# vinits5/bullet-envs

Measured on AMD Instinct MI355X. Metric: env-steps/sec (whole node), 16-link snake, 4096 envs/GPU, higher is better.
Workload: dtype f32

## Files before the change

### bullet-envs_amd/csrc/snk_dynamics.hpp

```cpp
#pragma once
#include "snk_lds.hpp"
#include "snk_model.hpp"
#include "snk_wave.hpp"

namespace snk {

template <class LT>
__device__ void fk_vel(LT& L, const DevModel& M, int lane) {
    constexpr int N = LT::kN;
    const float* bs = L.base();
    float qx = bs[3], qy = bs[4], qz = bs[5], qw = bs[6];
    float dd = qx * qx + qy * qy + qz * qz + qw * qw;
    float s2 = 2.0f / dd;
    float xs = qx * s2, ys = qy * s2, zs = qz * s2;
    float wx = qw * xs, wy = qw * ys, wz = qw * zs;
    float xx = qx * xs, xy = qx * ys, xz = qx * zs, yy = qy * ys, yz = qy * zs, zz = qz * zs;
    float Rp[9] = {1 - (yy + zz), xy - wz, xz + wy, xy + wz, 1 - (xx + zz), yz - wx, xz - wy, yz + wx, 1 - (xx + yy)};
    f3 op = ld3(bs), wp = ld3(bs + 7), vp = ld3(bs + 10);
    if (lane == 0) {
#pragma unroll
        for (int i = 0; i < 9; i++) L.R[0][i] = Rp[i];
        st3(L.o[0], op); st3(L.w[0], wp); st3(L.v[0], vp);
        st3(L.r[0], mk3(0, 0, 0)); st3(L.ax[0], mk3(0, 0, 0));
#pragma unroll
        for (int i = 0; i < 6; i++) L.zeta[0][i] = 0.f;
    }
    float snv = 0.f, csv = 1.f;
    if (lane < N) sincosf(L.q()[lane], &snv, &csv);
#pragma unroll 4
    for (int b = 1; b <= N; b++) {
        const float* Rf = M.Rfix[b];
        float T[9];
#pragma unroll
        for (int i = 0; i < 3; i++)
#pragma unroll
            for (int j = 0; j < 3; j++)
                T[3 * i + j] = Rp[3 * i] * Rf[j] + Rp[3 * i + 1] * Rf[3 + j] + Rp[3 * i + 2] * Rf[6 + j];
        float qdb = L.qd()[b - 1];
        const float sn = __int_as_float(__builtin_amdgcn_readlane(__float_as_int(snv), b - 1));
        const float cs = __int_as_float(__builtin_amdgcn_readlane(__float_as_int(csv), b - 1));
        float Rn[9];
#pragma unroll
        for (int i = 0; i < 3; i++) {
            Rn[3 * i + 0] = cs * T[3 * i] - sn * T[3 * i + 2];
            Rn[3 * i + 1] = T[3 * i + 1];
            Rn[3 * i + 2] = sn * T[3 * i] + cs * T[3 * i + 2];
        }
        f3 rb = mulRv(Rp, ld3(M.pfix[b]));
        f3 o = op + rb;
        f3 ax = mk3(T[1], T[4], T[7]);
        f3 w = wp + ax * qdb;
        f3 v = vp + cross(wp, rb);
        f3 za = cross(wp, ax) * qdb;
        f3 zl = cross(wp, cross(wp, rb));
        if (lane == 0) {
#pragma unroll
            for (int i = 0; i < 9; i++) L.R[b][i] = Rn[i];
            st3(L.o[b], o); st3(L.r[b], rb); st3(L.ax[b], ax); st3(L.w[b], w); st3(L.v[b], v);
            st3(&L.zeta[b][0], za); st3(&L.zeta[b][3], zl);
        }
#pragma unroll
        for (int i = 0; i < 9; i++) Rp[i] = Rn[i];
        op = o; wp = w; vp = v;
    }
    lds_sync();
}

template <class LT>
__device__ float mean_height(LT& L, const DevModel& M, int lane) {
    constexpr int N = LT::kN;
    float z = 0.f;
    if (lane == 0) z = L.o[0][2] + L.R[0][6] * M.hbase[0] + L.R[0][7] * M.hbase[1] + L.R[0][8] * M.hbase[2];
    else if (lane <= N) z = L.o[lane][2];
    return wave_sum<64>(z) * (1.0f / (N + 1));
}

template <class LT, bool FIRST>
__device__ void body_bias(LT& L, const DevModel& M, int lane) {
    constexpr int N = LT::kN;
    if (lane <= N) {
        const int b = lane;
        const float* R = L.R[b];
        f3 w = ld3(L.w[b]), v = ld3(L.v[b]);
        float m = M.mass[b];
        f3 cw = mulRv(R, ld3(M.com[b]));
        float Ibar[6];
        rotSym(R, M.Ib[b], Ibar);
        f3 pN = cross(w, mulSv(Ibar, w));
        f3 pF = cross(w, cross(w, cw)) * m;
        float Irw[6];
        rotSym(R, M.Irot[b], Irw);
        float nw = sqrtf(dot(w, w));
        pN = pN + mulSv(Irw, w) * (M.ang_damp + M.ang_damp * nw);
        const int ns = M.nsub[b];
        for (int s = 0; s < ns; s++) {
            f3 cs = mulRv(R, ld3(M.sub_c[b][s]));
            f3 vs = v + cross(w, cs);
            float nv = sqrtf(dot(vs, vs));
            f3 F = vs * (M.sub_m[b][s] * (M.lin_damp + M.lin_damp * nv));
            pF = pF + F;
            pN = pN + cross(cs, F);
        }
        if (FIRST) {
            f3 G = mk3(0.f, 0.f, m * M.gz);
            pF = pF - G;
            pN = pN - cross(cw, G);
            st3(L.cw[b], cw);
            float* IA = L.IA[b];
#pragma unroll
            for (int i = 0; i < 6; i++) IA[i] = Ibar[i];
            float hx = m * cw.x, hy = m * cw.y, hz = m * cw.z;
            IA[6] = 0.f; IA[7] = -hz; IA[8] = hy;
            IA[9] = hz;  IA[10] = 0.f; IA[11] = -hx;
            IA[12] = -hy; IA[13] = hx; IA[14] = 0.f;
            IA[15] = m; IA[16] = 0.f; IA[17] = 0.f; IA[18] = m; IA[19] = 0.f; IA[20] = m;
        } else {
            pN = pN - ld3(L.ext(b));
            pF = pF - ld3(L.ext(b) + 3);
        }
        st3(&L.p[b][0], pN);
        st3(&L.p[b][3], pF);
    }
}

template <class LT, bool FACTOR>
__device__ void aba_main(LT& L, const DevModel& M, int lane) {
    constexpr int N = LT::kN;
    float cA[6], cB[9], cC[6];
#pragma unroll
    for (int i = 0; i < 6; i++) { cA[i] = 0.f; cC[i] = 0.f; }
#pragma unroll
    for (int i = 0; i < 9; i++) cB[i] = 0.f;
    f3 cN = mk3(0, 0, 0), cF = mk3(0, 0, 0);
    for (int b = N; b >= 1; b--) {
        float A[6], B[9], C[6];
        float* IA = L.IA[b];
#pragma unroll
        for (int i = 0; i < 6; i++) { A[i] = IA[i]; C[i] = IA[15 + i]; }
#pragma unroll
        for (int i = 0; i < 9; i++) B[i] = IA[6 + i];
        if (FACTOR) {
#pragma unroll
            for (int i = 0; i < 6; i++) { A[i] += cA[i]; C[i] += cC[i]; }
#pragma unroll
            for (int i = 0; i < 9; i++) B[i] += cB[i];
        }
        f3 pN = ld3(&L.p[b][0]) + cN, pF = ld3(&L.p[b][3]) + cF;
        f3 ax = ld3(L.ax[b]);
        f3 Ua, Ub;
        float Dinv;
        if (FACTOR) {
            Ua = mulSv(A, ax);
            Ub = mk3(B[0] * ax.x + B[3] * ax.y + B[6] * ax.z, B[1] * ax.x + B[4] * ax.y + B[7] * ax.z,
                     B[2] * ax.x + B[5] * ax.y + B[8] * ax.z);
            Dinv = 1.0f / dot(ax, Ua);
        } else {
            Ua = ld3(L.Ua[b]); Ub = ld3(L.Ub[b]); Dinv = L.Dinv[b];
        }
        f3 za = ld3(&L.zeta[b][0]), zl = ld3(&L.zeta[b][3]);
        float u = L.tauj[b - 1] - dot(ax, pN);
        f3 tN = mulSv(A, za) + mk3(B[0] * zl.x + B[1] * zl.y + B[2] * zl.z, B[3] * zl.x + B[4] * zl.y + B[5] * zl.z,
                                   B[6] * zl.x + B[7] * zl.y + B[8] * zl.z);
        f3 tF = mk3(B[0] * za.x + B[3] * za.y + B[6] * za.z, B[1] * za.x + B[4] * za.y + B[7] * za.z,
                    B[2] * za.x + B[5] * za.y + B[8] * za.z) + mulSv(C, zl);
        float uz = dot(Ua, za) + dot(Ub, zl);
        float s = (u - uz) * Dinv;
        f3 paN = pN + tN + Ua * s, paF = pF + tF + Ub * s;
        f3 r = ld3(L.r[b]);
        cN = paN + cross(r, paF);
        cF = paF;
        if (lane == 0) {
            L.u[b] = u;
            if (FACTOR) {
#pragma unroll
                for (int i = 0; i < 6; i++) { IA[i] = A[i]; IA[15 + i] = C[i]; }
#pragma unroll
                for (int i = 0; i < 9; i++) IA[6 + i] = B[i];
                st3(L.Ua[b], Ua); st3(L.Ub[b], Ub); L.Dinv[b] = Dinv;
            }
        }
        if (FACTOR) {
            float ua[3] = {Ua.x, Ua.y, Ua.z}, ub[3] = {Ub.x, Ub.y, Ub.z};
            float Ap[6], Bp[9], Cp[6];
            Ap[0] = A[0] - ua[0] * ua[0] * Dinv; Ap[1] = A[1] - ua[0] * ua[1] * Dinv; Ap[2] = A[2] - ua[0] * ua[2] * Dinv;
            Ap[3] = A[3] - ua[1] * ua[1] * Dinv; Ap[4] = A[4] - ua[1] * ua[2] * Dinv; Ap[5] = A[5] - ua[2] * ua[2] * Dinv;
            Cp[0] = C[0] - ub[0] * ub[0] * Dinv; Cp[1] = C[1] - ub[0] * ub[1] * Dinv; Cp[2] = C[2] - ub[0] * ub[2] * Dinv;
            Cp[3] = C[3] - ub[1] * ub[1] * Dinv; Cp[4] = C[4] - ub[1] * ub[2] * Dinv; Cp[5] = C[5] - ub[2] * ub[2] * Dinv;
#pragma unroll
            for (int i = 0; i < 3; i++)
#pragma unroll
                for (int j = 0; j < 3; j++) Bp[3 * i + j] = B[3 * i + j] - ua[i] * ub[j] * Dinv;
            f3 c0 = cross(r, mk3(Cp[0], Cp[1], Cp[2]));
            f3 c1 = cross(r, mk3(Cp[1], Cp[3], Cp[4]));
            f3 c2 = cross(r, mk3(Cp[2], Cp[4], Cp[5]));
            float Bn[9] = {Bp[0] + c0.x, Bp[1] + c1.x, Bp[2] + c2.x, Bp[3] + c0.y, Bp[4] + c1.y, Bp[5] + c2.y,
                           Bp[6] + c0.z, Bp[7] + c1.z, Bp[8] + c2.z};
            f3 e0 = cross(r, mk3(Bp[0], Bp[1], Bp[2])), e1 = cross(r, mk3(Bp[3], Bp[4], Bp[5])),
               e2 = cross(r, mk3(Bp[6], Bp[7], Bp[8]));
            f3 g0 = cross(r, mk3(Bn[0], Bn[1], Bn[2])), g1 = cross(r, mk3(Bn[3], Bn[4], Bn[5])),
               g2 = cross(r, mk3(Bn[6], Bn[7], Bn[8]));
            cA[0] = Ap[0] + e0.x + g0.x;
            cA[1] = Ap[1] + e0.y + g1.x;
            cA[2] = Ap[2] + e0.z + g2.x;
            cA[3] = Ap[3] + e1.y + g1.y;
            cA[4] = Ap[4] + e1.z + g2.y;
            cA[5] = Ap[5] + e2.z + g2.z;
#pragma unroll
            for (int i = 0; i < 9; i++) cB[i] = Bn[i];
#pragma unroll
            for (int i = 0; i < 6; i++) cC[i] = Cp[i];
        }
    }
    f3 pN = ld3(&L.p[0][0]) + cN, pF = ld3(&L.p[0][3]) + cF;
    float p0[6] = {pN.x, pN.y, pN.z, pF.x, pF.y, pF.z};
    if (FACTOR) {
        float* IA = L.IA[0];
        float A[6], B[9], C[6];
#pragma unroll
        for (int i = 0; i < 6; i++) { A[i] = IA[i] + cA[i]; C[i] = IA[15 + i] + cC[i]; }
#pragma unroll
        for (int i = 0; i < 9; i++) B[i] = IA[6 + i] + cB[i];
        float G[6][6];
        G[0][0] = A[0]; G[0][1] = A[1]; G[0][2] = A[2]; G[1][1] = A[3]; G[1][2] = A[4]; G[2][2] = A[5];
        G[1][0] = A[1]; G[2][0] = A[2]; G[2][1] = A[4];
        G[3][3] = C[0]; G[3][4] = C[1]; G[3][5] = C[2]; G[4][4] = C[3]; G[4][5] = C[4]; G[5][5] = C[5];
        G[4][3] = C[1]; G[5][3] = C[2]; G[5][4] = C[4];
#pragma unroll
        for (int i = 0; i < 3; i++)
#pragma unroll
            for (int j = 0; j < 3; j++) { G[i][3 + j] = B[3 * i + j]; G[3 + j][i] = B[3 * i + j]; }
        float V[6][6];
#pragma unroll
        for (int i = 0; i < 6; i++)
#pragma unroll
            for (int j = 0; j < 6; j++) V[i][j] = (i == j) ? 1.f : 0.f;
#pragma unroll
        for (int k = 0; k < 6; k++) {
            float piv = 1.0f / G[k][k];
#pragma unroll
            for (int j = 0; j < 6; j++) { G[k][j] *= piv; V[k][j] *= piv; }
#pragma unroll
            for (int i = 0; i < 6; i++) {
                if (i != k) {
                    float f = G[i][k];
#pragma unroll
                    for (int j = 0; j < 6; j++) { G[i][j] -= f * G[k][j]; V[i][j] -= f * V[k][j]; }
                }
            }
        }
        if (lane == 0) {
#pragma unroll
            for (int i = 0; i < 6; i++)
#pragma unroll
                for (int j = 0; j < 6; j++) L.Inv0[6 * i + j] = V[i][j];
        }
        float a0[6];
#pragma unroll
        for (int i = 0; i < 6; i++) {
            float s = 0.f;
#pragma unroll
            for (int j = 0; j < 6; j++) s -= V[i][j] * p0[j];
            a0[i] = s;
        }
        if (lane == 0) {
#pragma unroll
            for (int i = 0; i < 6; i++) L.acc0[i] = a0[i];
        }
    } else {
        float a0[6];
#pragma unroll
        for (int i = 0; i < 6; i++) {
            float s = 0.f;
#pragma unroll
            for (int j = 0; j < 6; j++) s -= L.Inv0[6 * i + j] * p0[j];
            a0[i] = s;
        }
        if (lane == 0) {
#pragma unroll
            for (int i = 0; i < 6; i++) L.acc0[i] = a0[i];
        }
    }
    lds_sync();
    if (!FACTOR) return;
    f3 al = ld3(&L.acc0[0]), a = ld3(&L.acc0[3]);
    for (int b = 1; b <= N; b++) {
        f3 r = ld3(L.r[b]);
        f3 ap = a + cross(al, r) + ld3(&L.zeta[b][3]);
        f3 alp = al + ld3(&L.zeta[b][0]);
        float qdd = (L.u[b] - (dot(ld3(L.Ua[b]), alp) + dot(ld3(L.Ub[b]), ap))) * L.Dinv[b];
        al = alp + ld3(L.ax[b]) * qdd;
        a = ap;
        if (lane == 0) L.qdd[b - 1] = qdd;
    }
    lds_sync();
}

template <class LT>
__device__ __forceinline__ bool sensor_pass_needed(LT& L, const DevModel& M, int lane, float dv, const SensorHint& hint) {
    constexpr int N = LT::kN;
    constexpr int ND = N + 6;
    if (hint.always) return true;
    const float dt = M.dt;
    float e = 0.f, wgt = 0.f;
    if (lane < ND) {
        const float vold = lane < 6 ? L.base()[7 + lane] : L.qd()[lane - 6];
        const float x = fminf(fmaxf(vold + dv, -M.max_vel), M.max_vel);
        if (lane >= 6) e = L.targets[lane - 6] - (L.q()[lane - 6] + dt * x);
        wgt = fabsf(x) * ((lane >= 3 && lane < 6) ? 1.0f : 0.0639f * (N + 2));
    }
    const float se = wave_sum<64>(e * e);
    const float reach = dt * wave_sum<64>(wgt);
    const float tol = M.servo_tol * 1.001f;
    const bool sensor = !(se > tol * tol) || hint.counter_next > M.max_counter || !(hint.h_prev + reach < M.height_thr);
    return __builtin_amdgcn_readfirstlane(sensor ? 1 : 0) != 0;
}

}
```

### bullet-envs_amd/csrc/snk_pgs_v2.hpp

```cpp
#pragma once
#include "snk_contacts.hpp"
#include "snk_dynamics.hpp"
#include "snk_lds.hpp"
#include "snk_model.hpp"
#include "snk_selfcol.hpp"
#include "snk_wave.hpp"

namespace snk {


constexpr int kSlotNormal = 0;
constexpr int kSlotFric = 32;
constexpr int kSlots = 96;
constexpr int kAppMotor = 0;
constexpr int kAppNormal = 16;
constexpr int kAppFric = 80;
constexpr unsigned long long kLowMask = 0x00000000FFFFFFFFull;


struct ObsHit {
    bool hit;
    f3 P, n, dA, dB;
    float dist;
};
// ... 522 lines not shown
        "v_readlane_b32 %[s0], %[RJ], 31\n\t"
        SNK_REDUCE_12
        "v_readlane_b32 %[s2], %[RJ], 63\n\t"
        "v_mov_b32 %[xA], %[s0]\n\t"
        SNK_REDUCE_22
        "v_mov_b32 %[xB], %[s2]\n\t"
        "s_nop 0\n\t"
        SNK_REDUCE_345
        "v_readlane_b32 %[s1], %[t], 31\n\t"
        "v_readlane_b32 %[s3], %[t], 63\n\t"
        "s_nop 0\n\t"
        "v_fma_f32 %[r2], %[s1], %[s1], 1\n\t"
        "v_fma_f32 %[r2], %[s3], %[s3], %[r2]\n\t"
        "v_rsq_f32 %[r2], %[r2]\n\t"
        "s_nop 0\n\t"
        "v_mul_f32_e64 %[r2], %[s4], %[r2] clamp\n\t"
        "v_fma_f32 %[xA], %[r2], -%[s1], -%[xA]\n\t"
        "v_fma_f32 %[xB], %[r2], -%[s3], -%[xB]\n\t"
        "v_cndmask_b32_e64 %[t], %[xB], %[xA], %[lowmask]\n\t"
        "v_mul_f32 %[r2], %[RM], %[t]\n\t"
        "v_mul_f32 %[c2], %[RM], %[t]\n\t"
        SNK_ACC3163("%[RJ]", "%[t]")
        "s_nop 0\n\t"
        "v_permlane32_swap_b32 %[r2], %[c2]\n\t"
        "v_add_f32 %[dv], %[dv], %[r2]\n\t"
        "v_add_f32 %[dv], %[dv], %[c2]\n\t"
        : [t] "=&v"(t), [xA] "=&v"(xA), [xB] "=&v"(xB), [r2] "=&v"(r2), [c2] "=&v"(c2),
          [s0] "=&s"(s0), [s1] "=&s"(s1), [s2] "=&s"(s2), [s3] "=&s"(s3), [s4] "=&s"(s4), [RJ] "+v"(RJ), [dv] "+v"(dv)
        : [RM] "v"(RM), [RJnorm] "v"(RJnorm), [lowmask] "s"(lowmask),
          [NLn] "n"(NL));
    if (RES) asm volatile("v_max3_f32 %[lsq], %[lsq], |%[r2]|, |%[c2]|" : [lsq] "+v"(lsq) : [r2] "v"(r2), [c2] "v"(c2));
}

#define SNK_STR_(x) #x
#define SNK_V1(a) "v" SNK_STR_(a)
#define SNK_S1(a) "s" SNK_STR_(a)
#define SNK_VP(a, b) "v[" SNK_STR_(a) ":" SNK_STR_(b) "]"
#define SNK_SP(a, b) "s[" SNK_STR_(a) ":" SNK_STR_(b) "]"
#define SNK_CONE2_BODY_(P0, P1, P2, P3, P4, P5, Q0, Q1, Q2, Q3, Q4, Q5) \
    "v_mul_f32 %[t1], %[RJ1], %[dv]\n\t" \
    "v_mul_f32 %[t2], %[RJ2], %[dv]\n\t" \
    "v_readlane_b32 " SNK_S1(Q0) ", %[RJ1], 31\n\t" \
    "v_readlane_b32 " SNK_S1(Q1) ", %[RJ1], 63\n\t" \
    SNK_RED2("quad_perm:[1,0,3,2] row_mask:0xf bank_mask:0xf bound_ctrl:1") \
    "v_readlane_b32 " SNK_S1(Q2) ", %[RJ2], 31\n\t" \
    "v_readlane_b32 " SNK_S1(Q3) ", %[RJ2], 63\n\t" \
    SNK_RED2("quad_perm:[2,3,0,1] row_mask:0xf bank_mask:0xf bound_ctrl:1") \
    "v_readlane_b32 %[l1], %[RJn], 31\n\t" \
    "v_readlane_b32 %[l2], %[RJn], 63\n\t" \
    SNK_RED2("row_shr:4 row_mask:0xf bank_mask:0xf bound_ctrl:1") \
    "v_mov_b64 " SNK_VP(P0, P1) ", " SNK_SP(Q0, Q1) "\n\t" \
    SNK_RED2("row_shr:8 row_mask:0xf bank_mask:0xf bound_ctrl:1") \
    "v_mov_b64 " SNK_VP(P2, P3) ", " SNK_SP(Q2, Q3) "\n\t" \
    SNK_RED2("row_bcast:15 row_mask:0xa bank_mask:0xf") \
    "v_readlane_b32 " SNK_S1(Q4) ", %[t1], 31\n\t" \
    "v_readlane_b32 " SNK_S1(Q5) ", %[t1], 63\n\t" \
    "s_nop 0\n\t" \
    "v_fma_f32 " SNK_V1(P4) ", " SNK_S1(Q4) ", " SNK_S1(Q4) ", 1\n\t" \
    "v_fma_f32 " SNK_V1(P4) ", " SNK_S1(Q5) ", " SNK_S1(Q5) ", " SNK_V1(P4) "\n\t" \
    "v_rsq_f32 " SNK_V1(P4) ", " SNK_V1(P4) "\n\t" \
    "s_nop 0\n\t" \
    "v_mul_f32_e64 " SNK_V1(P4) ", %[l1], " SNK_V1(P4) " clamp\n\t" \
    "v_pk_fma_f32 " SNK_VP(P0, P1) ", " SNK_VP(P4, P5) ", " SNK_SP(Q4, Q5) ", " SNK_VP(P0, P1) " op_sel_hi:[0,1,1] neg_lo:[0,1,1] neg_hi:[0,1,1]\n\t" \
    "v_fmac_f32_dpp %[t2], %[RJ2], " SNK_V1(P0) " row_shr:1 row_mask:0xf bank_mask:0xf bound_ctrl:1\n\t" \
    "v_fmac_f32_dpp %[t2], %[RJ2], " SNK_V1(P1) " row_shr:2 row_mask:0xf bank_mask:0xf bound_ctrl:1\n\t" \
    "v_cndmask_b32_e64 " SNK_V1(P0) ", " SNK_V1(P1) ", " SNK_V1(P0) ", %[lowmask]\n\t" \
    "v_readlane_b32 " SNK_S1(Q4) ", %[t2], 31\n\t" \
    "v_readlane_b32 " SNK_S1(Q5) ", %[t2], 63\n\t" \
    "v_mul_f32 " SNK_V1(P1) ", %[RM1], " SNK_V1(P0) "\n\t" \
    SNK_ACC3163("%[RJ1]", SNK_V1(P0)) \
    "v_fma_f32 " SNK_V1(P4) ", " SNK_S1(Q4) ", " SNK_S1(Q4) ", 1\n\t" \
    "v_fma_f32 " SNK_V1(P4) ", " SNK_S1(Q5) ", " SNK_S1(Q5) ", " SNK_V1(P4) "\n\t" \
    "v_rsq_f32 " SNK_V1(P4) ", " SNK_V1(P4) "\n\t" \
    "s_nop 0\n\t" \
    "v_mul_f32_e64 " SNK_V1(P4) ", %[l2], " SNK_V1(P4) " clamp\n\t" \
    "v_pk_fma_f32 " SNK_VP(P2, P3) ", " SNK_VP(P4, P5) ", " SNK_SP(Q4, Q5) ", " SNK_VP(P2, P3) " op_sel_hi:[0,1,1] neg_lo:[0,1,1] neg_hi:[0,1,1]\n\t" \
    "v_cndmask_b32_e64 " SNK_V1(P2) ", " SNK_V1(P3) ", " SNK_V1(P2) ", %[lowmask]\n\t" \
    "v_mul_f32 " SNK_V1(P3) ", %[RM2], " SNK_V1(P2) "\n\t"
#define SNK_CONE2_TAIL_(P0, P1, P2, P3, P4, P5, Q0, Q1, Q2, Q3, Q4, Q5)                           \
    "v_add_f32 " SNK_V1(P1) ", " SNK_V1(P1) ", " SNK_V1(P3) "\n\t"           \
    "v_mov_b32 " SNK_V1(P3) ", " SNK_V1(P1) "\n\t"                 \
    SNK_ACC3163("%[RJ2]", SNK_V1(P2))                \
    "s_nop 0\n\t"                              \
    "v_permlane32_swap_b32 " SNK_V1(P1) ", " SNK_V1(P3) "\n\t"     \
    "v_add_f32 %[dv], %[dv], " SNK_V1(P1) "\n\t"         \
    "v_add_f32 %[dv], %[dv], " SNK_V1(P3) "\n\t"
#define SNK_PINS_HI 250, 251, 252, 253, 254, 255, 84, 85, 86, 87, 88, 89
#define SNK_PINS_LO 162, 163, 164, 165, 166, 167, 84, 85, 86, 87, 88, 89
#define SNK_PINS_128 122, 123, 124, 125, 126, 127, 84, 85, 86, 87, 88, 89
#define SNK_CONE2_X(M_, ...) M_(__VA_ARGS__)
#define SNK_CONE2_ASM(RESLINE, PINS, CLOB)                                                                               \
    asm volatile(SNK_CONE2_X(SNK_CONE2_BODY_, PINS) RESLINE SNK_CONE2_X(SNK_CONE2_TAIL_, PINS)                              \
                 : [t1] "=&v"(t1), [t2] "=&v"(t2), [l1] "=&s"(l1), [l2] "=&s"(l2), [RJ1] "+v"(RJ1), [RJ2] "+v"(RJ2),       \
                   [dv] "+v"(dv), [lsq] "+v"(lsq)                                                                         \
                 : [RM1] "v"(RM1), [RM2] "v"(RM2), [RJn] "v"(RJnorm), [lowmask] "s"(lowmask)                             \
                 : CLOB, "s84", "s85", "s86", "s87", "s88", "s89")
template <bool RES, int PIN = 0>
__device__ __forceinline__ void cone2_step(float& RJ1, const float RM1, float& RJ2, const float RM2, const float RJnorm,
                                           float& dv, float EPS, float E3163, unsigned long long lowmask, float& lsq) {
    float t1, t2;
    float l1, l2;
#define SNK_CLOB_HI "v250", "v251", "v252", "v253", "v254", "v255"
#define SNK_CLOB_LO "v162", "v163", "v164", "v165", "v166", "v167"
#define SNK_CLOB_128 "v122", "v123", "v124", "v125", "v126", "v127"
    if constexpr (PIN == 0) {
        if (RES) SNK_CONE2_ASM("v_max3_f32 %[lsq], %[lsq], |v251|, |v253|\n\t", SNK_PINS_HI, SNK_CLOB_HI);
        else SNK_CONE2_ASM("", SNK_PINS_HI, SNK_CLOB_HI);
    } else if constexpr (PIN == 1) {
        if (RES) SNK_CONE2_ASM("v_max3_f32 %[lsq], %[lsq], |v163|, |v165|\n\t", SNK_PINS_LO, SNK_CLOB_LO);
        else SNK_CONE2_ASM("", SNK_PINS_LO, SNK_CLOB_LO);
    } else {
        if (RES) SNK_CONE2_ASM("v_max3_f32 %[lsq], %[lsq], |v123|, |v125|\n\t", SNK_PINS_128, SNK_CLOB_128);
        else SNK_CONE2_ASM("", SNK_PINS_128, SNK_CLOB_128);
    }
}

template <int SH = 1>
__device__ __forceinline__ void cone2_coupling(const float RM1, float& RJ2, int lane) {
    const swap2 sw = half_swap(RM1, RM1);
    const float tA = half_reduce(RJ2 * sw.a);
    const float tB = half_reduce(RJ2 * sw.b);
    const float mA = __int_as_float(__builtin_amdgcn_update_dpp(0, __float_as_int(tA), 0x100 + SH, 0xf, 0xf, true));
    const float mB = __int_as_float(__builtin_amdgcn_update_dpp(0, __float_as_int(tB), 0x100 + SH + 1, 0xf, 0xf, true));
    const int d = lane & 31;
    RJ2 = d == 31 - SH ? mA : (d == 30 - SH ? mB : RJ2);
}

template <int J, bool CLAMP>
__device__ __forceinline__ float motor_step(const float RMj, float& dv, const float TARGV, float& ACCV, float PMIV) {
    float u, xs, s;
    unsigned long long sv;
    if (CLAMP) {
        asm volatile(
            "v_sub_f32 %[u], %[TARGV], %[dv]\n\t"
            "v_add_f32 %[xs], %[ACCV], %[u]\n\t"
            "v_med3_f32 %[xs], %[xs], -%[PMIV], %[PMIV]\n\t"
            "v_sub_f32 %[u], %[xs], %[ACCV]\n\t"
            "s_nop 0\n\t"
            "v_readlane_b32 %[s], %[u], %[LN]\n\t"
            "s_mov_b64 %[sv], exec\n\t"
            "s_mov_b64 exec, %[MASK]\n\t"
            "v_add_f32 %[ACCV], %[ACCV], %[u]\n\t"
            "s_mov_b64 exec, %[sv]\n\t"
            "v_fmac_f32 %[dv], %[s], %[RMj]\n\t"
            : [u] "=&v"(u), [xs] "=&v"(xs), [s] "=&s"(s), [sv] "=&s"(sv), [ACCV] "+v"(ACCV), [dv] "+v"(dv)
            : [RMj] "v"(RMj), [TARGV] "v"(TARGV), [PMIV] "v"(PMIV), [LN] "n"(6 + J), [MASK] "n"(1 << (6 + J)));
    } else {
        asm volatile(
            "v_sub_f32 %[u], %[TARGV], %[dv]\n\t"
            "s_nop 0\n\t"
            "v_readlane_b32 %[s], %[u], %[LN]\n\t"
            "s_mov_b64 %[sv], exec\n\t"
            "s_mov_b64 exec, %[MASK]\n\t"
            "v_add_f32 %[ACCV], %[ACCV], %[u]\n\t"
            "s_mov_b64 exec, %[sv]\n\t"
            "v_fmac_f32 %[dv], %[s], %[RMj]\n\t"
            : [u] "=&v"(u), [s] "=&s"(s), [sv] "=&s"(sv), [ACCV] "+v"(ACCV), [dv] "+v"(dv)
            : [RMj] "v"(RMj), [TARGV] "v"(TARGV), [LN] "n"(6 + J), [MASK] "n"(1 << (6 + J)));
        (void)xs;
    }
    return s;
}


template <bool RES, int BASE>
__device__ __forceinline__ void duos4(float (&RJ)[kSlots], float (&RM)[kSlots], float& dv, float E3163, float& lsq, int ncl) {
    quad_step<RES>(RJ[BASE], RM[BASE], RJ[BASE + 1], RM[BASE + 1], dv, E3163, kLowMask, lsq);
    if (ncl > 2 * (BASE - kSlotNormal) + 4)
        quad_step<RES>(RJ[BASE + 2], RM[BASE + 2], RJ[BASE + 3], RM[BASE + 3], dv, E3163, kLowMask, lsq);
}

template <bool RES, int G>
__device__ __forceinline__ void cones8(float (&RJ)[kSlots], float (&RM)[kSlots], float& dv, float EPS,
                                       float E3163, float& lsq, int ncl) {
#define SNK_CONE2(I)                                                                                                  \
    cone2_step<RES>(RJ[kSlotFric + 8 * G + 2 * (I)], RM[kSlotFric + 8 * G + 2 * (I)], RJ[kSlotFric + 8 * G + 2 * (I) + 1],   \
                    RM[kSlotFric + 8 * G + 2 * (I) + 1], RJ[kSlotNormal + 4 * G + (I)], dv, EPS, E3163, kLowMask, lsq);
    SNK_CONE2(0)
    SNK_CONE2(1)
    if (ncl > 8 * G + 4) {
        SNK_CONE2(2)
        SNK_CONE2(3)
    }
#undef SNK_CONE2
}

template <bool FWD, bool CLAMP, bool ALIVE, int NCO, class LT, int... K>
__device__ __forceinline__ float motors16_ordered(LT& L, const float (&RMm)[16], float& dv, const float TARGV, float& ACCV,
                                                  float PMIV, std::integer_sequence<int, K...>) {
    float res = 0.f;
    auto step = [&](auto j_c) {
        constexpr int J = decltype(j_c)::value;
        float s_ = motor_step<J, CLAMP>(RMm[J], dv, TARGV, ACCV, PMIV);
        res = fmaxf(res, fabsf(ALIVE ? s_ : s_ * (L.MmS[J][1] * L.MmS[J][2])));
    };
    (step(std::integral_constant<int, NoncontactOrder<16>::motor(FWD, K)>{}), ...);
    return res;
}
template <bool FWD, bool CLAMP, bool ALIVE, class LT>
__device__ __forceinline__ float motors16(LT& L, const float (&RMm)[16], float& dv, const float TARGV, float& ACCV,
                                          float PMIV) {
    if constexpr (LT::kNCO != 0)
        return motors16_ordered<FWD, CLAMP, ALIVE, LT::kNCO>(L, RMm, dv, TARGV, ACCV, PMIV,
                                                             std::make_integer_sequence<int, 16>{});
    float res = 0.f;
#define SNK_MOTOR(J)                                                                              \
    {                                                                                              \
        float s_ = motor_step<J, CLAMP>(RMm[J], dv, TARGV, ACCV, PMIV);                            \
        res = fmaxf(res, fabsf(ALIVE ? s_ : s_ * (L.MmS[J][1] * L.MmS[J][2])));                    \
    }
    if (FWD) {
        SNK_MOTOR(0) SNK_MOTOR(1) SNK_MOTOR(2) SNK_MOTOR(3) SNK_MOTOR(4) SNK_MOTOR(5) SNK_MOTOR(6) SNK_MOTOR(7)
        SNK_MOTOR(8) SNK_MOTOR(9) SNK_MOTOR(10) SNK_MOTOR(11) SNK_MOTOR(12) SNK_MOTOR(13) SNK_MOTOR(14) SNK_MOTOR(15)
    } else {
        SNK_MOTOR(15) SNK_MOTOR(14) SNK_MOTOR(13) SNK_MOTOR(12) SNK_MOTOR(11) SNK_MOTOR(10) SNK_MOTOR(9) SNK_MOTOR(8)
        SNK_MOTOR(7) SNK_MOTOR(6) SNK_MOTOR(5) SNK_MOTOR(4) SNK_MOTOR(3) SNK_MOTOR(2) SNK_MOTOR(1) SNK_MOTOR(0)
    }
#undef SNK_MOTOR
    return res;
}

template <bool RES>
__device__ __forceinline__ void contact_rows(float (&RJ)[kSlots], float (&RM)[kSlots], float& dv, int ncl, bool cone,
                                             float EPS, float E3163, float& lsq) {
    if (ncl > 0) duos4<RES, kSlotNormal + 0>(RJ, RM, dv, E3163, lsq, ncl);
    if (ncl > 8) duos4<RES, kSlotNormal + 4>(RJ, RM, dv, E3163, lsq, ncl);
    if (ncl > 16) duos4<RES, kSlotNormal + 8>(RJ, RM, dv, E3163, lsq, ncl);
    if (ncl > 24) duos4<RES, kSlotNormal + 12>(RJ, RM, dv, E3163, lsq, ncl);
    if (ncl > 32) duos4<RES, kSlotNormal + 16>(RJ, RM, dv, E3163, lsq, ncl);
    if (ncl > 40) duos4<RES, kSlotNormal + 20>(RJ, RM, dv, E3163, lsq, ncl);
    if (ncl > 48) duos4<RES, kSlotNormal + 24>(RJ, RM, dv, E3163, lsq, ncl);
    if (ncl > 56) duos4<RES, kSlotNormal + 28>(RJ, RM, dv, E3163, lsq, ncl);
    if (cone) {
        if (ncl > 0) cones8<RES, 0>(RJ, RM, dv, EPS, E3163, lsq, ncl);
        if (ncl > 8) cones8<RES, 1>(RJ, RM, dv, EPS, E3163, lsq, ncl);
        if (ncl > 16) cones8<RES, 2>(RJ, RM, dv, EPS, E3163, lsq, ncl);
        if (ncl > 24) cones8<RES, 3>(RJ, RM, dv, EPS, E3163, lsq, ncl);
        if (ncl > 32) cones8<RES, 4>(RJ, RM, dv, EPS, E3163, lsq, ncl);
        if (ncl > 40) cones8<RES, 5>(RJ, RM, dv, EPS, E3163, lsq, ncl);
        if (ncl > 48) cones8<RES, 6>(RJ, RM, dv, EPS, E3163, lsq, ncl);
        if (ncl > 56) cones8<RES, 7>(RJ, RM, dv, EPS, E3163, lsq, ncl);
    } else {
#pragma unroll
        for (int g = 0; g < 8; g++) {
            if (ncl > 8 * g) {
#pragma unroll
                for (int ci = 8 * g; ci < 8 * g + 8; ci++) {
                    float lim = rdlane(RJ[kSlotNormal + (ci >> 1)], (ci & 1) ? 63 : 31);
                    if (__builtin_amdgcn_readfirstlane(lim > 0.f ? 1 : 0))
                        duo_step<RES, true>(RJ[kSlotFric + ci], RM[kSlotFric + ci], dv, lim, E3163, kLowMask, lsq);
                }
            }
        }
    }
}

template <class LT>
__device__ __noinline__ void sensor_pass_v2(LT& L, const DevModel& M, const int nc, const int nlim
#ifdef SNK_PROFILE
                                            , unsigned long long* prof_t
#endif
) {
    constexpr int N = LT::kN;
    const int lane = lane_id();
    if (lane < nc) {
        const int ci = lane, k = L.ccbody[ci];
        const f3 nrm = ci < L.nplane ? mk3(0.f, 0.f, 1.f) : ld3(L.obn[ci - L.nplane]);
        f3 F = (nrm * L.app[kAppNormal + ci] +
                ld3(L.cdir[L.ccds[ci]][0]) * L.app[kAppFric + 2 * ci] +
                ld3(L.cdir[L.ccds[ci]][1]) * L.app[kAppFric + 2 * ci + 1]) * M.inv_dt;
        st3(&L.stM[ci][0], cross(ld3(L.ccP[ci]) - ld3(L.o[k]), F));
        st3(&L.stM[ci][3], F);
    }
    lds_sync();
    if (lane <= N) {
        const int b = lane;
        f3 eN = mk3(0, 0, 0), eF = mk3(0, 0, 0);
        const int c0 = b == 0 ? 0 : 2 * b - 1;
        const int ncyl = (b == 0 || b == N) ? 1 : 2;
        for (int cc = c0; cc < c0 + ncyl; cc++) {
            const int cb = L.cylbase[cc], cn = L.cyln[cc];
            for (int ci = cb; ci < cb + cn; ci++) {
                eN = eN + ld3(&L.stM[ci][0]);
                eF = eF + ld3(&L.stM[ci][3]);
            }
        }
        for (int ci = L.nplane; ci < nc; ci++)
            if (L.ccbody[ci] == b) {
                eN = eN + ld3(&L.stM[ci][0]);
                eF = eF + ld3(&L.stM[ci][3]);
            }
        st3(L.ext(b), eN);
        st3(L.ext(b) + 3, eF);
    }
    if (lane < N) L.tauj[lane] = -M.joint_damp * L.qd_old[lane] + L.app[lane] * M.inv_dt;
    lds_sync();
    if (lane == 0) {
        for (int i = 0; i < nlim; i++) L.tauj[L.nc_joint[i]] += L.nc_sign[i] * L.nc_app[i] * M.inv_dt;
    }
    lds_sync();
    {
        f3 wp = ld3(L.base() + 7), vp = ld3(L.base() + 10);
        if (lane == 0) { st3(L.w[0], wp); st3(L.v[0], vp); }
        for (int b = 1; b <= N; b++) {
            f3 ax = ld3(L.ax[b]), rb = ld3(L.r[b]);
            float qdb = L.qd()[b - 1];
            f3 w = wp + ax * qdb, v = vp + cross(wp, rb);
            f3 za = cross(wp, ax) * qdb, zl = cross(wp, cross(wp, rb));
            if (lane == 0) { st3(L.w[b], w); st3(L.v[b], v); st3(&L.zeta[b][0], za); st3(&L.zeta[b][3], zl); }
            wp = w; vp = v;
        }
    }
    lds_sync();
    SNK_STAMP(14)
    body_bias<LT, false>(L, M, lane);
    lds_sync();
    aba_main<LT, false>(L, M, lane);
    {
        f3 zb = mulRv(L.R[0], ld3(M.zbase));
        f3 v1 = ld3(L.base() + 10);
        float nv1 = sqrtf(dot(v1, v1));
        f3 a2 = ld3(&L.acc0[3]);
        const float fz = L.fz_park - dot(zb, a2 * M.m_root + v1 * (M.m_root * (M.lin_damp + M.lin_damp * nv1)));
        const f3 al2 = ld3(&L.acc0[0]);
        const f3 F3 = -((a2 + cross(al2, ld3(L.cw[0]))) * M.mass[0] + ld3(&L.p[0][3]));
        const float fz3 = L.fz3_park + F3.x * L.R[1][2] + F3.y * L.R[1][5] + F3.z * L.R[1][8];
        if (lane == 0) { L.fz() = fz; L.fz3() = fz3; }
    }
    SNK_STAMP(15)
}

template <class LT>
__device__ __forceinline__ void substep_v2(LT& L, const DevModel& M, int lane_in, float mu, int& iters, int& ncontacts,
                                           const SensorHint& hint, unsigned long long* __restrict__ ovf) {
    int lane = lane_in;
    constexpr int N = LT::kN;
    constexpr int ND = N + 6;
    static_assert(N == 16, "v2 is laid out for the 16-link chain");
    const float dt = M.dt;
#ifdef SNK_PROFILE
    unsigned long long prof_t[17];
#endif
    SNK_STAMP(0)
    const int nc = __builtin_amdgcn_readfirstlane(find_contacts_v2(L, M, lane, ovf));
    ncontacts = nc;
    if (nc < 0) return;
    SNK_STAMP(1)
    if (lane < N) {
        float qd = L.qd()[lane];
        L.qd_old[lane] = qd;
        L.tauj[lane] = -M.joint_damp * qd;
    }
    body_bias<LT, true>(L, M, lane);
    lds_sync();
    aba_main<LT, true>(L, M, lane);
    SNK_STAMP(2)
    {
        f3 zb = mulRv(L.R[0], ld3(M.zbase));
        f3 v_old = ld3(L.base() + 10);
        float nv0 = sqrtf(dot(v_old, v_old));
        f3 a1 = ld3(&L.acc0[3]);
        float fz1 = -dot(zb, (a1 - mk3(0.f, 0.f, M.gz)) * M.m_root + v_old * (M.m_root * (M.lin_damp + M.lin_damp * nv0)));
        const f3 al0 = ld3(&L.acc0[0]);
        const f3 F3 = -((a1 + cross(al0, ld3(L.cw[0]))) * M.mass[0] + ld3(&L.p[0][3]));
        if (lane == 0) { L.fz_park = fz1; L.fz3_park = F3.x * L.R[1][2] + F3.y * L.R[1][5] + F3.z * L.R[1][8]; }
    }
    if (lane < 6) {
        float x = L.base()[7 + lane] + L.acc0[lane] * dt;
        L.base()[7 + lane] = fminf(fmaxf(x, -M.max_vel), M.max_vel);
    } else if (lane < ND) {
        float x = L.qd()[lane - 6] + L.qdd[lane - 6] * dt;
        L.qd()[lane - 6] = fminf(fmaxf(x, -M.max_vel), M.max_vel);
    }
    lds_sync();

    SNK_STAMP(3)
    float RJ[kSlots], RM[kSlots];
    float RMm[16], TARGV;
    bool malive;
    float wsum = 0.f;
    {
        LaneK K;
        K.h = lane >> 5;
        K.d = lane & 31;
        K.isdof = K.d < ND;
        K.m22 = K.d == 22 ? -1.0f : 0.0f;
        K.m24 = K.d == 24 ? 1.0f : 0.0f;
        K.m31 = K.d == 31 ? 1.0f : 0.0f;
        K.spoff = K.d == 24 ? 1 : 0;
        K.bL = (K.d >= 6 && K.isdof) ? K.d - 5 : 0;
        K.oL = ld3(L.o[K.bL]);
        K.aL = (K.d >= 6 && K.isdof) ? ld3(L.ax[K.bL])
                                     : mk3(K.d == 0 ? 1.f : 0.f, K.d == 1 ? 1.f : 0.f, K.d == 2 ? 1.f : 0.f);
        MuScale ms;
        auto sgpr = [](float x) { return __int_as_float(__builtin_amdgcn_readfirstlane(__float_as_int(x))); };
        ms.fJ = sgpr(mu > 0.f ? 1.0f / mu : 0.f); ms.fM = sgpr(mu > 0.f ? mu : 0.f);
        const float mu_ob = fminf(M.mu_link * M.mu_obs, 10.0f);
        ms.fJo = sgpr(mu_ob > 0.f ? 1.0f / mu_ob : 0.f); ms.fMo = sgpr(mu_ob > 0.f ? mu_ob : 0.f);
        ms.nplane = __builtin_amdgcn_readfirstlane(L.nplane);
        build_batch_v2<LT, 0>(L, M, lane, nc);
        SNK_STAMP(4)
#pragma unroll
        for (int s = 0; s < kSlots - kSlotFric; s++) { RJ[kSlotFric + s] = 0.f; RM[kSlotFric + s] = 0.f; }
        build_batch_v2<LT, 4>(L, M, lane, nc, 0);
        SNK_STAMP(5)
        if (nc > 0) load_slots8<LT, 4, 0, kSlotFric>(L, K, nc, 0, ms, RJ, RM, wsum);
        if (nc > 8) load_slots8<LT, 4, 8, kSlotFric>(L, K, nc, 0, ms, RJ, RM, wsum);
        if (nc > 16) load_slots8<LT, 4, 16, kSlotFric>(L, K, nc, 0, ms, RJ, RM, wsum);
        if (nc > 24) load_slots8<LT, 4, 24, kSlotFric>(L, K, nc, 0, ms, RJ, RM, wsum);
        lds_sync();
        SNK_STAMP(6)
        if (nc > 32) {
            build_batch_v2<LT, 4>(L, M, lane, nc, 32);
            SNK_STAMP(7)
            load_slots8<LT, 4, 32, kSlotFric>(L, K, nc, 32, ms, RJ, RM, wsum);
            if (nc > 40) load_slots8<LT, 4, 40, kSlotFric>(L, K, nc, 32, ms, RJ, RM, wsum);
            if (nc > 48) load_slots8<LT, 4, 48, kSlotFric>(L, K, nc, 32, ms, RJ, RM, wsum);
            if (nc > 56) load_slots8<LT, 4, 56, kSlotFric>(L, K, nc, 32, ms, RJ, RM, wsum);
            lds_sync();
        } else {
            SNK_STAMP(7)
        }
        SNK_STAMP(8)
        build_batch_v2<LT, 1>(L, M, lane, nc);
        SNK_STAMP(9)
#pragma unroll
        for (int s = 0; s < kSlotFric; s++) { RJ[kSlotNormal + s] = 0.f; RM[kSlotNormal + s] = 0.f; }
        if (nc > 0) load_slots8<LT, 1, 0, kSlotNormal>(L, K, nc, 0, ms, RJ, RM, wsum);
        if (nc > 16) load_slots8<LT, 1, 8, kSlotNormal>(L, K, nc, 0, ms, RJ, RM, wsum);
        if (nc > 32) load_slots8<LT, 1, 16, kSlotNormal>(L, K, nc, 0, ms, RJ, RM, wsum);
        if (nc > 48) load_slots8<LT, 1, 24, kSlotNormal>(L, K, nc, 0, ms, RJ, RM, wsum);
#pragma unroll
        for (int j = 0; j < 16; j++) RMm[j] = K.isdof ? L.Mm[j][K.d] * L.MmS[j][2] : 0.f;
        {
            const bool mot = K.d >= 6 && K.isdof;
            const int jm = mot ? K.d - 6 : 0;
            const float dinv_m = mot ? L.MmS[jm][2] : 0.f;
            TARGV = (mot && dinv_m > 0.f) ? L.MmS[jm][3] : 0.f;
            malive = __all(!mot || dinv_m > 0.f) != 0;
        }
        lds_sync();
    }

    SNK_STAMP(10)
    {
#pragma unroll
        for (int g = 0; g < 8; g++) {
            if (nc > 8 * g) {
#pragma unroll
                for (int i = 0; i < 4; i++) {
                    const int s = kSlotNormal + 4 * g + i;
                    swap2 sw = half_swap(RM[s], RM[s]);
                    float t = half_reduce(RJ[s] * sw.a);
                    RJ[s] = wrlane(RJ[s], rdlane(t, 63), 62);
                }
#pragma unroll
                for (int i = 0; i < 2; i++) {
                    const int s = kSlotNormal + 4 * g + 2 * i;
                    cone2_coupling<2>(RM[s], RJ[s + 1], lane);
                }
            }
        }
        if (M.cone == 0) {
#pragma unroll
            for (int g = 0; g < 8; g++) {
                if (nc > 8 * g) {
#pragma unroll
                    for (int i = 0; i < 8; i++) {
                        const int s = kSlotFric + 8 * g + i;
                        swap2 sw = half_swap(RM[s], RM[s]);
                        float t = half_reduce(RJ[s] * sw.a);
                        RJ[s] = wrlane(RJ[s], rdlane(t, 63), 62);
                    }
                }
            }
        } else {
#pragma unroll
            for (int g = 0; g < 8; g++) {
                if (nc > 8 * g) {
#pragma unroll
                    for (int i = 0; i < 4; i++) {
                        const int s = kSlotFric + 8 * g + 2 * i;
                        cone2_coupling(RM[s], RJ[s + 1], lane);
                    }
                }
            }
        }
    }

    SNK_STAMP(11)
    int nlim = 0;
    {
        bool viol = false;
        float sgn = 0.f, pen = 0.f;
        if (lane < N) {
            float qj = L.q()[lane];
            float plo = qj - M.jlo, phi = M.jhi - qj;
            if (plo <= 0.f) { viol = true; sgn = 1.f; pen = plo; }
            else if (phi <= 0.f) { viol = true; sgn = -1.f; pen = phi; }
        }
        unsigned long long bal = __ballot(viol);
        nlim = __builtin_amdgcn_readfirstlane(__popcll(bal));
        if (viol) {
            unsigned long long before = (1ull << lane) - 1ull;
            if constexpr (LT::kNCO != 0) before = NoncontactOrder<N>::tab.below[lane];
            int idx = __popcll(bal & before);
            float den = L.Mm[lane][6 + lane];
            float dinv = den > 1.1920929e-7f ? 1.0f / den : 0.f;
            float rel = sgn * L.qd()[lane];
            L.nc_joint[idx] = lane; L.nc_sign[idx] = sgn;
            L.nc_rhs[idx] = (-rel + (-pen) * M.limit_erp * M.inv_dt) * dinv;
            L.nc_dinv[idx] = dinv; L.nc_den[idx] = den;
            L.nc_lo[idx] = 0.f; L.nc_hi[idx] = M.limit_max; L.nc_app[idx] = 0.f;
        }
        if (nlim) lds_sync();
    }

    SNK_STAMP(12)
    __builtin_amdgcn_s_setprio(3);
    float dv;
    {
        const int d = lane & 31;
        dv = d == 22 ? 1.0f : (d == 31 ? -1.0f : 0.0f);
        {
            const swap2 sw = half_swap(wsum, wsum);
            dv += sw.a + sw.b;
        }
        const float E3163 = d == 31 ? 1.0f : 0.0f;
        const float EPS = 1e-30f;
        const float mi = M.max_motor_imp;
        const bool mclamp = mi < 1e30f;
        float ACCV = 0.f;
        const float thr = __int_as_float(__builtin_amdgcn_readfirstlane(__float_as_int(sqrtf(M.resid_thr))));
        const int n_iter = M.n_iter;
        const bool cone = M.cone != 0;
        int it = 0;
#pragma unroll
        for (int s2 = 0; s2 < kSlots; s2++) asm volatile("" : "+v"(RJ[s2]), "+v"(RM[s2]));
#pragma unroll
        for (int j2 = 0; j2 < 16; j2++) asm volatile("" : "+v"(RMm[j2]));
        for (; it < n_iter; it++) {
            int exceeded = 0;
            int ncl = nc;
            asm volatile("" : "+s"(ncl));
#pragma unroll
            for (int s2 = 0; s2 < kSlots; s2++) asm volatile("" : "+v"(RJ[s2]), "+v"(RM[s2]));
            auto limit_rows = [&](bool fwd) {
                for (int jj = 0; jj < nlim; jj++) {
                    const int idx = fwd ? jj : nlim - 1 - jj;
                    const int j = __builtin_amdgcn_readfirstlane(L.nc_joint[idx]);
                    const float sg = L.nc_sign[idx];
                    float un = sg * rdlane(dv, 6 + j);
                    float a0 = L.nc_app[idx];
                    float dI = L.nc_rhs[idx] - un * L.nc_dinv[idx];
                    float sum = fminf(fmaxf(a0 + dI, L.nc_lo[idx]), L.nc_hi[idx]);
                    dI = sum - a0;
                    L.nc_app[idx] = sum;
                    float mv = (d < ND) ? L.Mm[j][d] : 0.f;
                    dv += sg * mv * dI;
                    if (__builtin_amdgcn_readfirstlane(fabsf(dI * L.nc_den[idx]) > thr ? 1 : 0)) exceeded = 1;
                }
            };
            float mres;
            auto pmiv = [&]() {
                const bool mot = d >= 6 && d < ND;
                const float dinv_m = mot ? L.MmS[mot ? d - 6 : 0][2] : 0.f;
                return (dinv_m > 0.f) ? mi / dinv_m : 1e30f;
            };
#define SNK_MOTORS(FWD)                                                                             \
    mres = malive ? (mclamp ? motors16<FWD, true, true>(L, RMm, dv, TARGV, ACCV, pmiv())             \
                            : motors16<FWD, false, true>(L, RMm, dv, TARGV, ACCV, 0.f))              \
                  : (mclamp ? motors16<FWD, true, false>(L, RMm, dv, TARGV, ACCV, pmiv())            \
                            : motors16<FWD, false, false>(L, RMm, dv, TARGV, ACCV, 0.f));
            if constexpr (LT::kNCO == 0) {
                if (it & 1) {
                    limit_rows(true);
                    SNK_MOTORS(true)
                } else {
                    SNK_MOTORS(false)
                    limit_rows(false);
                }
            } else {
                if (it & 1) {
                    SNK_MOTORS(true)
                    limit_rows(true);
                } else {
                    limit_rows(false);
                    SNK_MOTORS(false)
                }
            }
#undef SNK_MOTORS
            if (__builtin_amdgcn_readfirstlane(mres > thr ? 1 : 0)) exceeded = 1;
            {
                float l_ = 0.f;
                contact_rows<true>(RJ, RM, dv, ncl, cone, EPS, E3163, l_);
                float m = fmaxf(rdlane(l_, 24), rdlane(l_, 56));
                if (__builtin_amdgcn_readfirstlane(m > thr ? 1 : 0)) exceeded = 1;
            }
            if (!exceeded || it >= n_iter - 1) { it++; break; }
        }
        iters = it;
        lane = lane_id();
        if ((lane & 31) == 31) {
            const int h = lane >> 5;
#pragma unroll
            for (int s = 0; s < kSlotFric; s++) L.app[kAppNormal + 2 * s + h] = RJ[kSlotNormal + s];
            const int npl = L.nplane;
            const float mu_ob = fminf(M.mu_link * M.mu_obs, 10.0f);
#pragma unroll
            for (int s = 0; s < kSlots - kSlotFric; s++) L.app[kAppFric + 2 * s + h] = RJ[kSlotFric + s] * (s < npl ? mu : mu_ob);
        }
        if (lane >= 6 && lane < ND) L.app[kAppMotor + lane - 6] = ACCV * L.MmS[lane - 6][2];
    }
// ... 71 lines not shown
```

Before: 370,100.

## Prefetch next body's LDS data in ABA sweeps and tighten sensor-skip bound

The backward and forward articulated-body sweeps, and the velocity recursion, now load the next body's LDS data (inertia, bias forces, axes, zeta terms) into registers while the current body is computed. The goal is to hide LDS latency on the serial per-link chain. Joint velocities are also broadcast with readlane from one per-lane load instead of being re-read from LDS every iteration. In the V2 path, the sensor-skip check uses a tighter height-reach estimate weighted by each joint's horizontal axis and lever arm, so the sensor pass should be skipped more often. That new bound could be less conservative than the old one, and the prefetched registers raise register pressure.

After: 371,500, median of 6. Within noise of the previous version (+0.4%).

```diff
diff --git a/bullet-envs_amd/csrc/snk_dynamics.hpp b/bullet-envs_amd/csrc/snk_dynamics.hpp
--- a/bullet-envs_amd/csrc/snk_dynamics.hpp
+++ b/bullet-envs_amd/csrc/snk_dynamics.hpp
@@ -25,8 +25,8 @@
 #pragma unroll
         for (int i = 0; i < 6; i++) L.zeta[0][i] = 0.f;
     }
-    float snv = 0.f, csv = 1.f;
-    if (lane < N) sincosf(L.q()[lane], &snv, &csv);
+    float snv = 0.f, csv = 1.f, qdv = 0.f;
+    if (lane < N) { sincosf(L.q()[lane], &snv, &csv); qdv = L.qd()[lane]; }
 #pragma unroll 4
     for (int b = 1; b <= N; b++) {
         const float* Rf = M.Rfix[b];
@@ -36,7 +36,7 @@
 #pragma unroll
             for (int j = 0; j < 3; j++)
                 T[3 * i + j] = Rp[3 * i] * Rf[j] + Rp[3 * i + 1] * Rf[3 + j] + Rp[3 * i + 2] * Rf[6 + j];
-        float qdb = L.qd()[b - 1];
+        const float qdb = LT::kV2 ? __int_as_float(__builtin_amdgcn_readlane(__float_as_int(qdv), b - 1)) : L.qd()[b - 1];
         const float sn = __int_as_float(__builtin_amdgcn_readlane(__float_as_int(snv), b - 1));
         const float cs = __int_as_float(__builtin_amdgcn_readlane(__float_as_int(csv), b - 1));
         float Rn[9];
@@ -123,6 +123,38 @@
     }
 }
 
+template <bool FACTOR>
+struct AbaBodyK {
+    float IA[21];
+    f3 pN, pF, ax, za, zl, r, Ua, Ub;
+    float tauj, Dinv;
+};
+template <class LT, bool FACTOR>
+__device__ __forceinline__ AbaBodyK<FACTOR> load_aba_k(LT& L, int b) {
+    AbaBodyK<FACTOR> c;
+#pragma unroll
+    for (int i = 0; i < 21; i++) c.IA[i] = L.IA[b][i];
+    c.pN = ld3(&L.p[b][0]); c.pF = ld3(&L.p[b][3]);
+    c.ax = ld3(L.ax[b]);
+    if (!FACTOR) { c.Ua = ld3(L.Ua[b]); c.Ub = ld3(L.Ub[b]); c.Dinv = L.Dinv[b]; }
+    c.za = ld3(&L.zeta[b][0]); c.zl = ld3(&L.zeta[b][3]);
+    c.tauj = L.tauj[b > 0 ? b - 1 : 0];
+    c.r = ld3(L.r[b]);
+    return c;
+}
+struct AbaFwdK {
+    f3 r, za, zl, Ua, Ub, ax;
+    float u, Dinv;
+};
+template <class LT>
+__device__ __forceinline__ AbaFwdK load_aba_fwd_k(LT& L, int b) {
+    AbaFwdK c;
+    c.r = ld3(L.r[b]); c.za = ld3(&L.zeta[b][0]); c.zl = ld3(&L.zeta[b][3]);
+    c.Ua = ld3(L.Ua[b]); c.Ub = ld3(L.Ub[b]); c.ax = ld3(L.ax[b]);
+    c.u = L.u[b]; c.Dinv = L.Dinv[b];
+    return c;
+}
+
 template <class LT, bool FACTOR>
 __device__ void aba_main(LT& L, const DevModel& M, int lane) {
     constexpr int N = LT::kN;
@@ -132,21 +164,23 @@
 #pragma unroll
     for (int i = 0; i < 9; i++) cB[i] = 0.f;
     f3 cN = mk3(0, 0, 0), cF = mk3(0, 0, 0);
-    for (int b = N; b >= 1; b--) {
+    constexpr bool AHEAD = LT::kV2;
+    AbaBodyK<FACTOR> cur;
+    auto body = [&](const int b) {
         float A[6], B[9], C[6];
         float* IA = L.IA[b];
 #pragma unroll
-        for (int i = 0; i < 6; i++) { A[i] = IA[i]; C[i] = IA[15 + i]; }
-#pragma unroll
-        for (int i = 0; i < 9; i++) B[i] = IA[6 + i];
+        for (int i = 0; i < 6; i++) { A[i] = cur.IA[i]; C[i] = cur.IA[15 + i]; }
+#pragma unroll
+        for (int i = 0; i < 9; i++) B[i] = cur.IA[6 + i];
         if (FACTOR) {
 #pragma unroll
             for (int i = 0; i < 6; i++) { A[i] += cA[i]; C[i] += cC[i]; }
 #pragma unroll
             for (int i = 0; i < 9; i++) B[i] += cB[i];
         }
-        f3 pN = ld3(&L.p[b][0]) + cN, pF = ld3(&L.p[b][3]) + cF;
-        f3 ax = ld3(L.ax[b]);
+        f3 pN = cur.pN + cN, pF = cur.pF + cF;
+        f3 ax = cur.ax;
         f3 Ua, Ub;
         float Dinv;
         if (FACTOR) {
@@ -155,10 +189,10 @@
                      B[2] * ax.x + B[5] * ax.y + B[8] * ax.z);
             Dinv = 1.0f / dot(ax, Ua);
         } else {
-            Ua = ld3(L.Ua[b]); Ub = ld3(L.Ub[b]); Dinv = L.Dinv[b];
-        }
-        f3 za = ld3(&L.zeta[b][0]), zl = ld3(&L.zeta[b][3]);
-        float u = L.tauj[b - 1] - dot(ax, pN);
+            Ua = cur.Ua; Ub = cur.Ub; Dinv = cur.Dinv;
+        }
+        f3 za = cur.za, zl = cur.zl;
+        float u = cur.tauj - dot(ax, pN);
         f3 tN = mulSv(A, za) + mk3(B[0] * zl.x + B[1] * zl.y + B[2] * zl.z, B[3] * zl.x + B[4] * zl.y + B[5] * zl.z,
                                    B[6] * zl.x + B[7] * zl.y + B[8] * zl.z);
         f3 tF = mk3(B[0] * za.x + B[3] * za.y + B[6] * za.z, B[1] * za.x + B[4] * za.y + B[7] * za.z,
@@ -166,7 +200,7 @@
         float uz = dot(Ua, za) + dot(Ub, zl);
         float s = (u - uz) * Dinv;
         f3 paN = pN + tN + Ua * s, paF = pF + tF + Ub * s;
-        f3 r = ld3(L.r[b]);
+        f3 r = cur.r;
         cN = paN + cross(r, paF);
         cF = paF;
         if (lane == 0) {
@@ -210,11 +244,26 @@
 #pragma unroll
             for (int i = 0; i < 6; i++) cC[i] = Cp[i];
         }
-    }
-    f3 pN = ld3(&L.p[0][0]) + cN, pF = ld3(&L.p[0][3]) + cF;
+    };
+    if constexpr (AHEAD) {
+        cur = load_aba_k<LT, FACTOR>(L, N);
+#pragma unroll 2
+        for (int b = N; b >= 1; b--) {
+            const AbaBodyK<FACTOR> nxt = load_aba_k<LT, FACTOR>(L, b - 1);
+            body(b);
+            cur = nxt;
+        }
+    } else {
+        for (int b = N; b >= 1; b--) {
+            cur = load_aba_k<LT, FACTOR>(L, b);
+            body(b);
+        }
+        cur = load_aba_k<LT, FACTOR>(L, 0);
+    }
+    f3 pN = cur.pN + cN, pF = cur.pF + cF;
     float p0[6] = {pN.x, pN.y, pN.z, pF.x, pF.y, pF.z};
     if (FACTOR) {
-        float* IA = L.IA[0];
+        const float* IA = cur.IA;
         float A[6], B[9], C[6];
 #pragma unroll
         for (int i = 0; i < 6; i++) { A[i] = IA[i] + cA[i]; C[i] = IA[15 + i] + cC[i]; }
@@ -283,14 +332,28 @@
     lds_sync();
     if (!FACTOR) return;
     f3 al = ld3(&L.acc0[0]), a = ld3(&L.acc0[3]);
-    for (int b = 1; b <= N; b++) {
-        f3 r = ld3(L.r[b]);
-        f3 ap = a + cross(al, r) + ld3(&L.zeta[b][3]);
-        f3 alp = al + ld3(&L.zeta[b][0]);
-        float qdd = (L.u[b] - (dot(ld3(L.Ua[b]), alp) + dot(ld3(L.Ub[b]), ap))) * L.Dinv[b];
-        al = alp + ld3(L.ax[b]) * qdd;
+    AbaFwdK fw;
+    auto fwd = [&](const int b) {
+        f3 ap = a + cross(al, fw.r) + fw.zl;
+        f3 alp = al + fw.za;
+        float qdd = (fw.u - (dot(fw.Ua, alp) + dot(fw.Ub, ap))) * fw.Dinv;
+        al = alp + fw.ax * qdd;
         a = ap;
         if (lane == 0) L.qdd[b - 1] = qdd;
+    };
+    if constexpr (AHEAD) {
+        fw = load_aba_fwd_k(L, 1);
+#pragma unroll 4
+        for (int b = 1; b <= N; b++) {
+            const AbaFwdK fn = load_aba_fwd_k(L, b < N ? b + 1 : N);
+            fwd(b);
+            fw = fn;
+        }
+    } else {
+        for (int b = 1; b <= N; b++) {
+            fw = load_aba_fwd_k(L, b);
+            fwd(b);
+        }
     }
     lds_sync();
 }
@@ -305,13 +368,25 @@
     if (lane < ND) {
         const float vold = lane < 6 ? L.base()[7 + lane] : L.qd()[lane - 6];
         const float x = fminf(fmaxf(vold + dv, -M.max_vel), M.max_vel);
-        if (lane >= 6) e = L.targets[lane - 6] - (L.q()[lane - 6] + dt * x);
-        wgt = fabsf(x) * ((lane >= 3 && lane < 6) ? 1.0f : 0.0639f * (N + 2));
+        const float second = 0.5f * dt * x * x;
+        if constexpr (!LT::kV2) {
+            if (lane >= 6) e = L.targets[lane - 6] - (L.q()[lane - 6] + dt * x);
+            wgt = fabsf(x) * ((lane >= 3 && lane < 6) ? 1.0f : 0.0639f * (N + 2));
+        } else if (lane >= 6) {
+            const int j = lane - 5;
+            e = L.targets[lane - 6] - (L.q()[lane - 6] + dt * x);
+            const float ah = sqrtf(L.ax[j][0] * L.ax[j][0] + L.ax[j][1] * L.ax[j][1]);
+            wgt = (0.0639f * (float)((N - j) * (N - j + 1)) / (float)(2 * (N + 1))) * (fabsf(x) * ah + second);
+        } else if (lane < 3) {
+            wgt = (0.0639f * (0.5f * N + 1.0f)) * ((lane < 2 ? fabsf(x) : 0.f) + second);
+        } else if (lane == 5) {
+            wgt = fabsf(x);
+        }
     }
     const float se = wave_sum<64>(e * e);
-    const float reach = dt * wave_sum<64>(wgt);
+    const float rise = LT::kV2 ? 1.01f * dt * wave_sum<64>(wgt) + 1e-6f : dt * wave_sum<64>(wgt);
     const float tol = M.servo_tol * 1.001f;
-    const bool sensor = !(se > tol * tol) || hint.counter_next > M.max_counter || !(hint.h_prev + reach < M.height_thr);
+    const bool sensor = !(se > tol * tol) || hint.counter_next > M.max_counter || !(hint.h_prev + rise < M.height_thr);
     return __builtin_amdgcn_readfirstlane(sensor ? 1 : 0) != 0;
 }
 
diff --git a/bullet-envs_amd/csrc/snk_pgs_v2.hpp b/bullet-envs_amd/csrc/snk_pgs_v2.hpp
--- a/bullet-envs_amd/csrc/snk_pgs_v2.hpp
+++ b/bullet-envs_amd/csrc/snk_pgs_v2.hpp
@@ -848,13 +848,18 @@
     {
         f3 wp = ld3(L.base() + 7), vp = ld3(L.base() + 10);
         if (lane == 0) { st3(L.w[0], wp); st3(L.v[0], vp); }
+        f3 ax = ld3(L.ax[1]), rb = ld3(L.r[1]);
+        float qdb = L.qd()[0];
+#pragma unroll 4
         for (int b = 1; b <= N; b++) {
-            f3 ax = ld3(L.ax[b]), rb = ld3(L.r[b]);
-            float qdb = L.qd()[b - 1];
+            const int bn = b < N ? b + 1 : N;
+            const f3 axn = ld3(L.ax[bn]), rbn = ld3(L.r[bn]);
+            const float qdn = L.qd()[bn - 1];
             f3 w = wp + ax * qdb, v = vp + cross(wp, rb);
             f3 za = cross(wp, ax) * qdb, zl = cross(wp, cross(wp, rb));
             if (lane == 0) { st3(L.w[b], w); st3(L.v[b], v); st3(&L.zeta[b][0], za); st3(&L.zeta[b][3], zl); }
             wp = w; vp = v;
+            ax = axn; rb = rbn; qdb = qdn;
         }
     }
     lds_sync();
```
